# MecatronicaUSB/uw-slam

Hardware: AMD Instinct MI355X
Metric: frame-pair alignments/sec (640x480, 4 pyr lvls) (higher is better)
Workload: dtype f32; 1 GPU; synthetic 640x480 pairs, 4 pyramid levels (0..3), 10 GN iterations/level, no early exit, dense points, u16 depth plane, 1024 pairs in total, 1024 resident on rank 0 (128 distinct), image pyramids of both frames + depth pyramid and gradients of the reference frame + alignment per step; normal_equation_accumulation=f64, weights=identity, tuning=defaults, sampler=nearest, total_pairs=1024, pairs_on_rank0=1024

## Files before the change

### uw-slam_amd/csrc/uwt_kernels.h

```cpp
#pragma once

#include <hip/hip_runtime.h>
#include <stdint.h>

#include <type_traits>

#include "uwt_math.h"

namespace uwt {

constexpr int kBlock = 256;
constexpr int kAccFloats = 27;
constexpr int kRecWords = 64;
constexpr int kMaxSlices = 160;

constexpr int kArithOpenCV = 0, kArithLegacy = 1;

struct LevelK {
  int pitch;
  int iw, ih;
  int gw, gh;
  int n;
  int ng;
  float fx, fy, cx, cy, invfx, invfy;
// ... 903 lines not shown
};

__device__ __forceinline__ float sample_bilinear(const uint8_t* __restrict__ I2, const LevelK& L, float x, float y) {
  const float x0 = floorf(x), y0 = floorf(y);
  const float ax = x - x0, ay = y - y0;
  int ix0, iy0;
  asm("v_cvt_i32_f32 %0, %1" : "=v"(ix0) : "v"(x0));
  asm("v_cvt_i32_f32 %0, %1" : "=v"(iy0) : "v"(y0));
  asm("v_med3_i32 %0, %0, 0, %1" : "+v"(ix0) : "s"(L.iw - 1));
  asm("v_med3_i32 %0, %0, 0, %1" : "+v"(iy0) : "s"(L.ih - 1));
  const int ix1 = min(ix0 + 1, L.iw - 1), iy1 = min(iy0 + 1, L.ih - 1);
  const uint32_t r0 = __umul24((unsigned)iy0, (unsigned)L.pitch), r1 = __umul24((unsigned)iy1, (unsigned)L.pitch);
  const float a = (float)I2[r0 + (unsigned)ix0], b = (float)I2[r0 + (unsigned)ix1];
  const float c = (float)I2[r1 + (unsigned)ix0], d = (float)I2[r1 + (unsigned)ix1];
  const float top = __builtin_fmaf(ax, b - a, a);
  const float bot = __builtin_fmaf(ax, d - c, c);
  return __builtin_fmaf(ay, bot - top, top);
}

template <bool FINITE = false>
__device__ __forceinline__ float robust_weight(int mode, float rf, float inv_mad) {
  if (mode == kWeightsTukeyRef) {
    const float b = 4.6851f;
    const float inv_b2 = (float)(1.0 / (double)(b * b));
    const float x = rf * inv_mad;
    if (fabsf(x) <= b) {
      const float t = (float)(1.0 - (double)((x * x) * inv_b2));
      return t * t;
    }
    return 0.f;
  }
  if (mode == kWeightsHuber) {
    const float k = 1.345f;
    const float ax = fabsf(rf * inv_mad);
    if constexpr (FINITE) return ax <= k ? 1.0f : div_by<float>(k, ax, refined_rcp<float>(ax));
    return ax <= k ? 1.0f : k / ax;
  }
  return 1.0f;
}

struct WeightEntry {
  double rwd;
  double e;
  float w;
  float pad[3];
};
static_assert(sizeof(WeightEntry) == 32, "one ds_read_b32 (w) and, later, one ds_read_b128 (rwd, e) per pixel");
constexpr int kWeightTabBytes = 511 * (int)sizeof(WeightEntry);

__device__ __forceinline__ void fill_weight_table(WeightEntry* __restrict__ tab, int mode, float inv_mad, float gain) {
  for (int i = threadIdx.x; i < 511; i += kBlock) {
    const float rf = (float)(i - 255);
    const float w = robust_weight(mode, rf, inv_mad);
    const float rw1 = rf * w;
    WeightEntry t;
    t.w = w; t.pad[0] = t.pad[1] = t.pad[2] = 0.f;
    t.rwd = (double)((rf * gain) * w);
    t.e = (double)rf * (double)rw1;
    tab[i] = t;
  }
}

static __global__ __launch_bounds__(1024) void k_robust_weights(const float* __restrict__ r, int n, int kind, float* __restrict__ w,
                                                         float* __restrict__ out_stats) {
  __shared__ unsigned int hist[256];
  __shared__ float s_med, s_mad;
  auto median_of_hist = [&]() {
    const float m = (float)(n / 2);
    unsigned int bin = 0;
    float med = -1.0f;
    for (int i = 0; i < 256 && med < 0.0f; ++i) {
      bin += hist[i];
      if ((float)bin > m) med = (float)i;
    }
    return med;
  };
  for (int pass = 0; pass < 2; pass++) {
    for (int i = threadIdx.x; i < 256; i += blockDim.x) hist[i] = 0;
    __syncthreads();
    for (int i = threadIdx.x; i < n; i += blockDim.x) {
      const float v = pass == 0 ? r[i] : fabsf(r[i] - s_med);
      int q = (int)rintf(v);
      q = q < 0 ? 0 : (q > 255 ? 255 : q);
      atomicAdd(&hist[q], 1u);
    }
    __syncthreads();
    if (threadIdx.x == 0) {
      const float med = median_of_hist();
      if (pass == 0) s_med = med; else s_mad = 1.4826f * med;
    }
    __syncthreads();
  }
  if (threadIdx.x == 0) { out_stats[0] = s_med; out_stats[1] = s_mad; }
  if (!w) return;
  float mad = s_mad;
  if (mad == 0.0f) mad = 1.0f;
  const float inv_mad = (float)(1.0 / (double)mad);
  for (int i = threadIdx.x; i < n; i += blockDim.x) w[i] = robust_weight(kind, r[i], inv_mad);
}

struct TailUpdate {
  unsigned int* tickets;
  PairState* state;
  int* active;
  int on;
  int k, max_iters, early_exit, general, legacy_solve;
  float epsilon, gain;
};

struct ResidualArgs {
  const uint8_t* img;
  const int16_t* gx;
  const int16_t* gy;
  const uint16_t* depth;
  const int* ref_slots;
  const int* tgt_slots;
  const PairState* state;
  Pose pose;
  LevelK L;
  float zf, af;
  int groups_per_block;
  int slices;
  int pair_base;
  uint32_t* partials;
  const PairScale* scale;
  float gain;
  float* dumpJ;
  float* dumpR;
  uint8_t* dumpV;
  float* dumpW;
  int typed_loads;
  int stream_planes;
  int probe;
  TailUpdate tail;
};

struct CoreOverride {
  int groups_per_block;
  uint32_t* rec;
  const PairScale* scale = nullptr;
};

typedef float f4v __attribute__((ext_vector_type(4)));
typedef int i4v __attribute__((ext_vector_type(4)));
template <int VEC>
struct RefGroup {
  uint8_t i1[VEC];
  int16_t gx[VEC], gy[VEC];
  uint16_t dp[VEC];
  f4v gx4, gy4, dp4;
};

constexpr int kLoadsPlain = 0, kLoadsStream = 1, kLoadsTyped = 2;
template <int VEC, bool DEPTH, bool COMPUTE_ONLY = false, int STREAM = 0>
__device__ __forceinline__ void load_group(RefGroup<VEC>& r, const uint8_t* __restrict__ I1, const int16_t* __restrict__ GX,
                                           const int16_t* __restrict__ GY, const uint16_t* __restrict__ DP, uint32_t idx) {
  constexpr bool FAKE_PLANES = COMPUTE_ONLY;
  if constexpr (FAKE_PLANES) {
#pragma unroll
    for (int j = 0; j < VEC; j++) { r.i1[j] = (uint8_t)(idx + j); r.gx[j] = (int16_t)(idx * 3 + j); r.gy[j] = (int16_t)(idx * 5 - j); r.dp[j] = (uint16_t)(4000 + (idx & 255)); }
    return;
  }
  if constexpr (VEC == 4) {
    const uint32_t o2 = idx * 2u;
    if constexpr ((STREAM & kLoadsStream) != 0) {
      *reinterpret_cast<uint32_t*>(r.i1) = __builtin_nontemporal_load(reinterpret_cast<const uint32_t*>(I1 + idx));
      *reinterpret_cast<u2v*>(r.gx) = __builtin_nontemporal_load(reinterpret_cast<const u2v*>(reinterpret_cast<const uint8_t*>(GX) + o2));
      *reinterpret_cast<u2v*>(r.gy) = __builtin_nontemporal_load(reinterpret_cast<const u2v*>(reinterpret_cast<const uint8_t*>(GY) + o2));
      if constexpr (DEPTH) *reinterpret_cast<u2v*>(r.dp) = __builtin_nontemporal_load(reinterpret_cast<const u2v*>(reinterpret_cast<const uint8_t*>(DP) + o2));
    } else {
      *reinterpret_cast<uint32_t*>(r.i1) = *reinterpret_cast<const uint32_t*>(I1 + idx);
      *reinterpret_cast<uint2*>(r.gx) = *reinterpret_cast<const uint2*>(reinterpret_cast<const uint8_t*>(GX) + o2);
      *reinterpret_cast<uint2*>(r.gy) = *reinterpret_cast<const uint2*>(reinterpret_cast<const uint8_t*>(GY) + o2);
      if constexpr (DEPTH) *reinterpret_cast<uint2*>(r.dp) = *reinterpret_cast<const uint2*>(reinterpret_cast<const uint8_t*>(DP) + o2);
    }
  } else {
#pragma unroll
    for (int j = 0; j < VEC; j++) {
      r.i1[j] = I1[idx + j]; r.gx[j] = GX[idx + j]; r.gy[j] = GY[idx + j];
      if constexpr (DEPTH) r.dp[j] = DP[idx + j];
    }
  }
}

__device__ __forceinline__ i4v make_rsrc(const void* p, uint32_t bytes) {
  const unsigned long long b = (unsigned long long)p;
  i4v r;
  r.x = __builtin_amdgcn_readfirstlane((int)(unsigned)b);
  r.y = __builtin_amdgcn_readfirstlane((int)(unsigned)(b >> 32));
  r.z = __builtin_amdgcn_readfirstlane((int)bytes);
  r.w = __builtin_amdgcn_readfirstlane(0x00027FAC);
  return r;
}
struct TypedPlanes { const uint8_t* I1; i4v gx, gy, dp; };
template <bool DEPTH, bool NT>
__device__ __forceinline__ void load_group_typed(RefGroup<4>& r, const TypedPlanes& P, uint32_t idx) {
  const uint32_t o2 = idx * 2u;
  uint32_t& w = *reinterpret_cast<uint32_t*>(r.i1);
  if constexpr (NT) {
    asm volatile("global_load_dword %0, %1, %2 nt" : "+v"(w) : "v"(idx), "s"(P.I1));
    asm volatile("tbuffer_load_format_xyzw %0, %1, %2, 0 format:[BUF_DATA_FORMAT_16_16_16_16,BUF_NUM_FORMAT_SSCALED] offen nt" : "+v"(r.gx4) : "v"(o2), "s"(P.gx));
    asm volatile("tbuffer_load_format_xyzw %0, %1, %2, 0 format:[BUF_DATA_FORMAT_16_16_16_16,BUF_NUM_FORMAT_SSCALED] offen nt" : "+v"(r.gy4) : "v"(o2), "s"(P.gy));
    if constexpr (DEPTH) asm volatile("tbuffer_load_format_xyzw %0, %1, %2, 0 format:[BUF_DATA_FORMAT_16_16_16_16,BUF_NUM_FORMAT_SSCALED] offen nt" : "+v"(r.dp4) : "v"(o2), "s"(P.dp));
  } else {
    asm volatile("global_load_dword %0, %1, %2" : "+v"(w) : "v"(idx), "s"(P.I1));
    asm volatile("tbuffer_load_format_xyzw %0, %1, %2, 0 format:[BUF_DATA_FORMAT_16_16_16_16,BUF_NUM_FORMAT_SSCALED] offen" : "+v"(r.gx4) : "v"(o2), "s"(P.gx));
    asm volatile("tbuffer_load_format_xyzw %0, %1, %2, 0 format:[BUF_DATA_FORMAT_16_16_16_16,BUF_NUM_FORMAT_SSCALED] offen" : "+v"(r.gy4) : "v"(o2), "s"(P.gy));
    if constexpr (DEPTH) asm volatile("tbuffer_load_format_xyzw %0, %1, %2, 0 format:[BUF_DATA_FORMAT_16_16_16_16,BUF_NUM_FORMAT_SSCALED] offen" : "+v"(r.dp4) : "v"(o2), "s"(P.dp));
  }
}
template <bool DEPTH>
__device__ __forceinline__ void wait_planes_typed(RefGroup<4>& r) {
  uint32_t& w = *reinterpret_cast<uint32_t*>(r.i1);
  if constexpr (DEPTH) asm volatile("s_waitcnt vmcnt(0)" : "+v"(w), "+v"(r.gx4), "+v"(r.gy4), "+v"(r.dp4));
  else asm volatile("s_waitcnt vmcnt(0)" : "+v"(w), "+v"(r.gx4), "+v"(r.gy4));
}

template <int AR, int VEC, bool DEPTH, bool UNIT_FACTORS, bool DUMP, typename AccT, bool SQUARE = false, int SAMPLER = 0, int WEIGHTS = 0,
          bool COMPUTE_ONLY = false, int EXT_LDS = 0, int STREAM = 0, bool RAGGED = false>
__device__ __forceinline__ void residual_core(const ResidualArgs& a, const int pair, const int slice, const Pose& pose,
                                              unsigned char* lds, const RefGroup<VEC>* first = nullptr, int ref_slot = -1,
                                              int tgt_slot = -1, const CoreOverride* ov = nullptr);

template <int VEC, bool DEPTH, bool COMPUTE_ONLY>
__device__ __forceinline__ void load_first_group(RefGroup<VEC>& rg, const ResidualArgs& a, int ref_slot, int slice) {
  const size_t ref_off = (size_t)ref_slot * a.L.n;
  const int n_groups = a.L.ng / VEC;
  const int g = slice * a.groups_per_block + (int)threadIdx.x;
  load_group<VEC, DEPTH, COMPUTE_ONLY>(rg, a.img + ref_off, a.gx + ref_off, a.gy + ref_off, DEPTH ? a.depth + ref_off : nullptr,
                                       (uint32_t)min(g, n_groups - 1) * VEC);
}

template <int AR, int VEC, bool DEPTH, bool UNIT_FACTORS, bool DUMP, typename AccT, bool SQUARE = false, int SAMPLER = 0, int WEIGHTS = 0,
          bool COMPUTE_ONLY = false, int STREAM = 0, bool RAGGED = false>
__device__ __forceinline__ bool residual_block(const ResidualArgs& a, const int pair, const int slice) {
  Pose pose;
  if constexpr (COMPUTE_ONLY) {
    pose_identity(pose);
  } else if (a.state) {
    const PairState st = a.state[pair];
    if (st.level_done || st.status) return false;
    pose = st.pose;
  } else {
    pose = a.pose;
  }
  residual_core<AR, VEC, DEPTH, UNIT_FACTORS, DUMP, AccT, SQUARE, SAMPLER, WEIGHTS, COMPUTE_ONLY, 0, STREAM, RAGGED>(a, pair, slice, pose, nullptr);
  return true;
}

template <int AR, int VEC, bool DEPTH, bool UNIT_FACTORS, bool DUMP, typename AccT, bool SQUARE, int SAMPLER, int WEIGHTS, bool COMPUTE_ONLY,
          int EXT_LDS, int STREAM, bool RAGGED>
__device__ __forceinline__ void residual_core(const ResidualArgs& a, const int pair, const int slice, const Pose& pose,
                                              unsigned char* lds, const RefGroup<VEC>* first, int ref_slot, int tgt_slot,
                                              const CoreOverride* ov) {
  const int a_groups_per_block = ov ? ov->groups_per_block : a.groups_per_block;
  const bool a_probe = ov ? false : a.probe != 0;
  constexpr bool MASKED = std::is_same<AccT, double>::value && !DUMP;
  WarpK K;
  constexpr bool TD_LDS = AR == kArithOpenCV && !DUMP;
  __shared__ __attribute__((aligned(16))) double s_td[TD_LDS ? 12 : 2];
  if constexpr (TD_LDS) {
    warp_setup<kArithLegacy>(pose, K);
    if (threadIdx.x == 0) {
#pragma unroll
      for (int i = 0; i < 12; i++) s_td[i] = (double)K.T[i];
    }
    __syncthreads();
  } else {
    warp_setup<AR>(pose, K);
  }
  const LevelK L = a.L;
  if (ref_slot < 0) {
    ref_slot = a.ref_slots[pair];
    tgt_slot = a.tgt_slots[pair];
  }
  const size_t ref_off = (size_t)ref_slot * L.n, tgt_off = (size_t)tgt_slot * L.n;
  const uint8_t* __restrict__ I1 = a.img + ref_off;
  const uint8_t* __restrict__ I2 = a.img + tgt_off;
  const int16_t* __restrict__ GX = a.gx + ref_off;
  const int16_t* __restrict__ GY = a.gy + ref_off;
  const uint16_t* __restrict__ DP = DEPTH ? a.depth + ref_off : nullptr;

  __shared__ unsigned long long s_probe[2];
  if (a_probe && threadIdx.x == 0) {
    s_probe[0] = __builtin_amdgcn_s_memtime();
    s_probe[1] = __builtin_amdgcn_s_memrealtime();
  }
  AccT acc[kAccFloats];
#pragma unroll
  for (int i = 0; i < kAccFloats; i++) acc[i] = (AccT)0;
  uint32_t sum_r2 = 0, n_valid_wave = 0;
  double r2d = 0.0;
  constexpr bool GENERAL = SAMPLER != 0 || WEIGHTS != 0;
  AccT err = (AccT)0;
  float inv_mad = 1.f;
  if constexpr (WEIGHTS != 0) inv_mad = ov ? ov->scale->inv_mad : a.scale[pair].inv_mad;
  constexpr bool TABLE = WEIGHTS != 0 && SAMPLER == 0 && !DUMP;
  static_assert(!TABLE || EXT_LDS == 0, "the weighted path reduces in its own LDS");
  __shared__ __attribute__((aligned(16))) unsigned char tlds[TABLE ? kReduceLdsBytes : 16];
  static_assert(!TABLE || kWeightTabBytes <= kReduceLdsBytes, "table fits the reduction image");
  if constexpr (TABLE) {
    fill_weight_table(reinterpret_cast<WeightEntry*>(tlds), WEIGHTS, inv_mad, a.gain);
    __syncthreads();
  }

  const int n_groups = L.ng / VEC;
  const int g_begin = slice * a_groups_per_block;
  const int g_end = min(g_begin + a_groups_per_block, n_groups);
  const int iters = (g_end - g_begin + kBlock - 1) / kBlock;

  RefGroup<VEC> rg;
  int g = g_begin + (int)threadIdx.x;
  constexpr bool TYPED = (STREAM & kLoadsTyped) != 0;
  constexpr bool NT = (STREAM & kLoadsStream) != 0;
  static_assert(!TYPED || (VEC == 4 && std::is_same<AccT, double>::value && !DUMP && !COMPUTE_ONLY && SAMPLER == 0 && WEIGHTS == 0),
                "typed plane loads: the identity path's production shape");
  TypedPlanes TP;
  if constexpr (TYPED) {
    TP.I1 = I1;
    TP.gx = make_rsrc(GX, (uint32_t)L.n * 2u);
    TP.gy = make_rsrc(GY, (uint32_t)L.n * 2u);
    TP.dp = make_rsrc(DEPTH ? (const void*)DP : (const void*)GX, (uint32_t)L.n * 2u);
    *reinterpret_cast<uint32_t*>(rg.i1) = 0u;
    rg.gx4 = rg.gy4 = rg.dp4 = (f4v)(0.f);
    load_group_typed<DEPTH, NT>(rg, TP, (uint32_t)min(g, n_groups - 1) * VEC);
  } else if (first) rg = *first;
  else load_group<VEC, DEPTH, COMPUTE_ONLY, STREAM>(rg, I1, GX, GY, DP, (uint32_t)min(g, n_groups - 1) * VEC);
  const uint32_t idx0 = (uint32_t)g * VEC;
  const uint32_t y0 = __umulhi(idx0, L.magic);
  float yf = (float)y0, xf0 = (float)(idx0 - y0 * (uint32_t)L.pitch);
  const uint32_t step_y = __umulhi((uint32_t)(kBlock * VEC), L.magic);
  const float step_yf = (float)step_y, step_xf = (float)((uint32_t)(kBlock * VEC) - step_y * (uint32_t)L.pitch), wf = (float)L.pitch;
  constexpr int N = (VEC % 2 == 0) ? 2 : 1;
  using F = typename std::conditional<N == 2, v2f, float>::type;
  constexpr int NU = VEC / N;
  auto body = [&](RefGroup<VEC>& rg, const int ahead, RefGroup<VEC>& nxt) __attribute__((always_inline)) {
    const bool active = g < g_end;
    const unsigned long long active_mask = __builtin_amdgcn_sicmp(g, g_end, kIcmpSLT);
    constexpr bool TD_READ = TD_LDS;
    if constexpr (TD_READ) {
      unsigned off = 0;
      asm volatile("" : "+v"(off));
      const double* tdp = reinterpret_cast<const double*>(reinterpret_cast<const unsigned char*>(s_td) + off);
#pragma unroll
      for (int i = 0; i < 12; i++) K.Td[i] = tdp[i];
    }
    const uint32_t idx = (uint32_t)min(g, n_groups - 1) * VEC;
    if constexpr (TYPED) wait_planes_typed<DEPTH>(rg);
    uint8_t i1[VEC];
#pragma unroll
    for (int j = 0; j < VEC; j++) i1[j] = rg.i1[j];
    F x2[NU], y2[NU], iz[NU];
    unsigned long long okm[VEC];
    uint32_t gidx[VEC];
    unsigned long long colm[VEC];
#pragma unroll
    for (int j = 0; j < VEC; j++) colm[j] = active_mask;
    if constexpr (RAGGED) {
      const unsigned long long m_in = active_mask & __builtin_amdgcn_fcmpf(xf0, (float)L.gw, kFcmpOLT);
      const unsigned long long m_all = active_mask & __builtin_amdgcn_fcmpf(xf0, (float)(L.gw & ~3), kFcmpOLT);
      const int rem = L.gw & 3;
#pragma unroll
      for (int j = 0; j < VEC; j++) colm[j] = (VEC == 1 || j < rem) ? m_in : m_all;
    }
#pragma unroll
    for (int u = 0; u < NU; u++) {
      F z = bc<F>(1.0f), xf;
      unsigned long long okin[N];
      float dlow[N];
#pragma unroll
      for (int c = 0; c < N; c++) {
        const int j = u * N + c;
        okin[c] = colm[j];
        dlow[c] = 1.0f;
        if constexpr (DEPTH && TYPED) {
          const float d = rg.dp4[j];
          dlow[c] = d;
          put(z, c, d);
        } else if constexpr (DEPTH) {
          const int d = (int)(int16_t)rg.dp[j];
          dlow[c] = (float)d;
          if constexpr (!MASKED) okin[c] &= __builtin_amdgcn_sicmp(d, 0, kIcmpSGT);
          put(z, c, dlow[c]);
        }
        put(xf, c, (float)j);
      }
      if constexpr (DEPTH) z = z * bc<F>(L.zscale);
      xf = bc<F>(xf0) + xf;
      if constexpr (MASKED) {
        if constexpr (DEPTH) {
          F z2;
          warp_point<AR, F>(L, K, xf, bc<F>(yf), z, x2[u], y2[u], z2, iz[u]);
#pragma unroll
          for (int c = 0; c < N; c++) {
            const float uc = get(x2[u], c), vc = get(y2[u], c);
            float lo;
            asm("v_min3_f32 %0, %1, %2, %3" : "=v"(lo) : "v"(uc), "v"(vc), "v"(dlow[c]));
            okm[u * N + c] = okin[c] & __builtin_amdgcn_fcmpf(lo, 0.f, kFcmpOGT) & __builtin_amdgcn_fcmpf(vc, (float)L.ih, kFcmpOLT) &
                             __builtin_amdgcn_fcmpf(uc, (float)L.iw, kFcmpOLT);
          }
        } else {
          pixel_warp_raw<AR, F>(L, K, xf, bc<F>(yf), z, okin, x2[u], y2[u], iz[u], &okm[u * N]);
        }
#pragma unroll
        for (int c = 0; c < N; c++) {
          float r = get(iz[u], c);
          asm("v_max_f32 %0, 0, %0" : "+v"(r));
          put(iz[u], c, r);
          int ix2 = round_pos(get(x2[u], c)), iy2 = round_pos(get(y2[u], c));
          asm("v_med3_i32 %0, %0, 0, %1" : "+v"(ix2) : "s"(L.iw - 1));
          asm("v_med3_i32 %0, %0, 0, %1" : "+v"(iy2) : "s"(L.ih - 1));
          gidx[u * N + c] = __umul24((unsigned)iy2, (unsigned)L.pitch) + (unsigned)ix2;
        }
      } else {
        pixel_warp<AR, F>(L, K, xf, bc<F>(yf), z, okin, x2[u], y2[u], iz[u], &okm[u * N], &gidx[u * N]);
      }
    }
    int i2[VEC];
    float s2[VEC];
#pragma unroll
    for (int j = 0; j < VEC; j++) {
      constexpr bool FAKE_GATHER = COMPUTE_ONLY;
      if constexpr (FAKE_GATHER) i2[j] = (int)i1[j] + (int)(gidx[j] & 1);
      else if constexpr (TYPED) asm volatile("global_load_ubyte %0, %1, %2" : "=v"(i2[j]) : "v"(gidx[j]), "s"(I2));
      else if constexpr (SAMPLER == 0) i2[j] = I2[gidx[j]];
      else s2[j] = sample_bilinear(I2, L, get(x2[j / N], j % N), get(y2[j / N], j % N));
    }
    F g0[NU], g1[NU];
#pragma unroll
    for (int j = 0; j < VEC; j++) {
      if constexpr (MASKED) {
        float gxf, gyf;
        if constexpr (TYPED) { gxf = rg.gx4[j]; gyf = rg.gy4[j]; }
        else { gxf = (float)rg.gx[j]; gyf = (float)rg.gy[j]; }
        if constexpr (AR == kArithOpenCV && !TYPED) {
          asm("" : "+v"(gxf));
          asm("" : "+v"(gyf));
        }
        put(g0[j / N], j % N, gxf);
        put(g1[j / N], j % N, gyf);
      } else {
        put(g0[j / N], j % N, keep_f((float)rg.gx[j], okm[j]));
        put(g1[j / N], j % N, keep_f((float)rg.gy[j], okm[j]));
      }
    }
    __builtin_amdgcn_sched_barrier(0);
    if constexpr (TYPED) load_group_typed<DEPTH, NT>(nxt, TP, (uint32_t)min(g + ahead * kBlock, n_groups - 1) * VEC);
    else load_group<VEC, DEPTH, COMPUTE_ONLY, STREAM>(nxt, I1, GX, GY, DP, (uint32_t)min(g + ahead * kBlock, n_groups - 1) * VEC);
    __builtin_amdgcn_sched_barrier(0);
    auto gathers_landed = [&]() __attribute__((always_inline)) {
      if constexpr (TYPED) asm volatile("s_waitcnt vmcnt(%4)" : "+v"(i2[0]), "+v"(i2[1]), "+v"(i2[2]), "+v"(i2[3]) : "n"(DEPTH ? 4 : 3));
    };
    constexpr bool DIRECT = AR == kArithOpenCV && MASKED && !GENERAL;
    if constexpr (DIRECT) {
#pragma unroll
      for (int u = 0; u < NU; u++) {
        F a0, b1, av[4], bv[4];
        jw_terms<UNIT_FACTORS, SQUARE, F>(L, a.zf, a.af, x2[u], y2[u], iz[u], a0, b1, av, bv);
        const F j0 = g0[u] * a0, j1 = g1[u] * b1;
#pragma unroll
        for (int c = 0; c < N; c++) {
          const int j = u * N + c;
          double Jd[6];
          jacobian_row_f64<SQUARE, F>(g0[u], g1[u], j0, j1, av, bv, c, Jd);
          if (u == 0 && c == 0) gathers_landed();
          const int ri = i2[j] - (int)i1[j];
          masked_sums_lo(acc, Jd, okm[j]);
          masked_sums_hi<0>(acc, r2d, Jd, (double)ri, 0.0, okm[j]);
          n_valid_wave += (uint32_t)__builtin_popcountll(okm[j]);
          __builtin_amdgcn_sched_barrier(0);
        }
      }
    } else if constexpr (MASKED && GENERAL && !TABLE) {
#pragma unroll
      for (int u = 0; u < NU; u++) {
        if constexpr (SAMPLER != 0) {
          if (u == 0) {
#pragma unroll
            for (int j = 0; j < VEC; j++) asm volatile("" : "+v"(s2[j]));
          }
        }
        F a0, b1, av[4], bv[4], j0, j1, Ju[6];
        if constexpr (AR == kArithOpenCV) {
          jw_terms<UNIT_FACTORS, SQUARE, F>(L, a.zf, a.af, x2[u], y2[u], iz[u], a0, b1, av, bv);
          j0 = g0[u] * a0;
          j1 = g1[u] * b1;
        } else {
          pixel_jacobian<AR, UNIT_FACTORS, SQUARE, false, F>(L, a.zf, a.af, x2[u], y2[u], iz[u], g0[u], g1[u], Ju);
        }
#pragma unroll
        for (int c = 0; c < N; c++) {
          const int j = u * N + c;
          float Jp[6];
          if constexpr (AR == kArithOpenCV) jacobian_row_f32<SQUARE, F>(g0[u], g1[u], j0, j1, av, bv, c, Jp);
          else {
#pragma unroll
            for (int k = 0; k < 6; k++) Jp[k] = get(Ju[k], c);
          }
          float rf;
          if constexpr (SAMPLER == 0) rf = (float)(i2[j] - (int)i1[j]);
          else rf = s2[j] - (float)i1[j];
          const float w = robust_weight<true>(WEIGHTS, rf, inv_mad);
          double Jd[6];
#pragma unroll
          for (int k = 0; k < 6; k++) Jd[k] = (double)(w * Jp[k]);
          const double e = (double)rf * (double)(rf * w);
          masked_sums_lo(acc, Jd, okm[j]);
          masked_sums_hi<1>(acc, err, Jd, (double)((rf * a.gain) * w), e, okm[j]);
          n_valid_wave += (uint32_t)__builtin_popcountll(okm[j]);
          __builtin_amdgcn_sched_barrier(0);
        }
      }
    } else {
    F J[NU][6];
#pragma unroll
    for (int u = 0; u < NU; u++)
      pixel_jacobian<AR, UNIT_FACTORS, SQUARE, DUMP, F>(L, a.zf, a.af, x2[u], y2[u], iz[u], g0[u], g1[u], J[u]);
    __builtin_amdgcn_sched_barrier(0);
    gathers_landed();
    if constexpr (TABLE) {
#pragma unroll
      for (int u = 0; u < NU; u++) {
        uint32_t off[N];
        F wv;
#pragma unroll
        for (int c = 0; c < N; c++) {
          const int j = u * N + c;
          const int ri = i2[j] - (int)i1[j];
          n_valid_wave += (uint32_t)__builtin_popcountll(okm[j]);
          off[c] = (uint32_t)(ri + 255) * (uint32_t)sizeof(WeightEntry);
          put(wv, c, *reinterpret_cast<const float*>(tlds + off[c] + 16));
        }
#pragma unroll
        for (int k = 0; k < 6; k++) J[u][k] = wv * J[u][k];
#pragma unroll
        for (int c = 0; c < N; c++) {
          const int j = u * N + c;
          const double2 re = *reinterpret_cast<const double2*>(tlds + off[c]);
          if constexpr (MASKED) {
            double Jd[6];
#pragma unroll
            for (int k = 0; k < 6; k++) Jd[k] = (double)get(J[u][k], c);
            masked_sums_lo(acc, Jd, okm[j]);
            masked_sums_hi<1>(acc, err, Jd, re.x, re.y, okm[j]);
          } else {
            float Jp[6];
#pragma unroll
            for (int k = 0; k < 6; k++) Jp[k] = get(J[u][k], c);
            const unsigned long long m = okm[j];
            if (lane_bit(m)) {
              err += (AccT)re.y;
              accumulate_preweighted(acc, Jp, re.x);
            }
          }
        }
        __builtin_amdgcn_sched_barrier(0);
      }
    } else {
#pragma unroll
    for (int j = 0; j < VEC; j++) {
      float Jp[6];
#pragma unroll
      for (int k = 0; k < 6; k++) Jp[k] = get(J[j / N][k], j % N);
      int ri = 0;
      float rf_dump = 0.f, w_dump = 0.f;
      if constexpr (!GENERAL && MASKED) {
        ri = i2[j] - (int)i1[j];
        double Jd[6];
#pragma unroll
        for (int k = 0; k < 6; k++) Jd[k] = (double)Jp[k];
        masked_sums_lo(acc, Jd, okm[j]);
        masked_sums_hi<0>(acc, r2d, Jd, (double)ri, 0.0, okm[j]);
      } else if constexpr (!GENERAL) {
        ri = keep_i(i2[j] - (int)i1[j], okm[j]);
        accumulate(acc, Jp, ri);
      } else if constexpr (MASKED) {
        float rf;
        if constexpr (SAMPLER == 0) rf = (float)(i2[j] - (int)i1[j]);
        else rf = s2[j] - (float)i1[j];
        const float w = robust_weight<true>(WEIGHTS, rf, inv_mad);
        double Jd[6];
#pragma unroll
        for (int k = 0; k < 6; k++) Jd[k] = (double)(w * Jp[k]);
        const double e = (double)rf * (double)(rf * w);
        masked_sums_lo(acc, Jd, okm[j]);
        masked_sums_hi<1>(acc, err, Jd, (double)((rf * a.gain) * w), e, okm[j]);
      } else {
        float rf;
        if constexpr (SAMPLER == 0) rf = (float)keep_i(i2[j] - (int)i1[j], okm[j]);
        else rf = keep_f(s2[j] - (float)i1[j], okm[j]);
        const float w = robust_weight(WEIGHTS, rf, inv_mad);
        accumulate_weighted(acc, err, Jp, rf, w, a.gain);
        ri = (int)rintf(rf);
        if constexpr (DUMP) {
          rf_dump = rf;
          w_dump = w;
        }
      }
      if constexpr (GENERAL || !MASKED) sum_r2 += (uint32_t)__mul24(ri, ri);
      n_valid_wave += (uint32_t)__builtin_popcountll(okm[j]);
      if constexpr (DUMP) {
        if (active) {
          const size_t p = (size_t)pair * L.ng + idx + j;
          const bool ok = lane_bit(okm[j]);
          if (a.dumpV) a.dumpV[p] = ok ? 1 : 0;
          if constexpr (GENERAL) {
            if (a.dumpR) a.dumpR[p] = ok ? rf_dump : 0.f;
            if (a.dumpW) a.dumpW[p] = ok ? w_dump : 0.f;
            if (a.dumpJ)
              for (int k = 0; k < 6; k++) a.dumpJ[p * 6 + k] = ok ? Jp[k] : 0.f;
          } else {
            if (a.dumpR) a.dumpR[p] = (float)ri;
            if (a.dumpJ)
              for (int k = 0; k < 6; k++) a.dumpJ[p * 6 + k] = Jp[k];
          }
        }
      }
    }
    }
    }
    xf0 += step_xf;
    yf += step_yf;
    const bool wrap = xf0 >= wf;
    xf0 -= wrap ? wf : 0.f;
    yf += wrap ? 1.f : 0.f;
  };
  if constexpr (TYPED) {
    RefGroup<VEC> rgB;
    *reinterpret_cast<uint32_t*>(rgB.i1) = 0u;
    rgB.gx4 = rgB.gy4 = rgB.dp4 = (f4v)(0.f);
    for (int it = 0; it < iters; it += 2) {
      body(rg, 1, rgB);
      g += kBlock;
      if (it + 1 < iters) {
        body(rgB, 1, rg);
        g += kBlock;
      }
    }
    wait_planes_typed<DEPTH>(rg);
    wait_planes_typed<DEPTH>(rgB);
  } else {
    for (int it = 0; it < iters; it++, g += kBlock) body(rg, 1, rg);
  }
  const uint32_t n_valid = (threadIdx.x & 63) == 0 ? n_valid_wave : 0u;
  uint32_t* out_rec = ov ? ov->rec : a.partials + ((size_t)pair * a.slices + slice) * kRecWords;
  constexpr bool R2D = MASKED && !GENERAL;
  const bool coherent = !ov && a.tail.on != 0;
  if constexpr (EXT_LDS != 0 && R2D) block_reduce_store_at<AccT, false, EXT_LDS, double>(lds, acc, r2d, n_valid, out_rec, err);
  else if constexpr (EXT_LDS != 0) block_reduce_store_at<AccT, GENERAL, EXT_LDS>(lds, acc, sum_r2, n_valid, out_rec, err);
  else if constexpr (TABLE) {
    __syncthreads();
    block_reduce_store_at<AccT, true>(tlds, acc, sum_r2, n_valid, out_rec, err, coherent);
  } else if constexpr (R2D) block_reduce_store<AccT, false, double>(acc, r2d, n_valid, out_rec, err, coherent);
  else block_reduce_store<AccT, GENERAL>(acc, sum_r2, n_valid, out_rec, err, coherent);
  if (a_probe && threadIdx.x == 0) {
    uint32_t* rec = a.partials + ((size_t)pair * a.slices + slice) * kRecWords;
    rec[60] = (uint32_t)(__builtin_amdgcn_s_memtime() - s_probe[0]);
    rec[61] = (uint32_t)(__builtin_amdgcn_s_memrealtime() - s_probe[1]);
  }
}

__device__ __forceinline__ void tail_update_wave(const ResidualArgs& a, int pair);

template <int AR, int VEC, bool DEPTH, bool UNIT_FACTORS, bool DUMP, typename AccT, bool SQUARE = false, int SAMPLER = 0, int WEIGHTS = 0,
          bool COMPUTE_ONLY = false, int STREAM = 0, bool RAGGED = false>
__global__ __launch_bounds__(kBlock) void k_residual(const ResidualArgs a) {
  const int pair = (int)blockIdx.y + a.pair_base;
  const bool live = residual_block<AR, VEC, DEPTH, UNIT_FACTORS, DUMP, AccT, SQUARE, SAMPLER, WEIGHTS, COMPUTE_ONLY, STREAM, RAGGED>(a, pair, (int)blockIdx.x);
  if constexpr (!COMPUTE_ONLY && !DUMP) {
    if (a.tail.on && live && threadIdx.x < 64) tail_update_wave(a, pair);
  }
}

template <int AR, int VEC, bool DEPTH, bool UNIT_FACTORS, bool DUMP, typename AccT, bool SQUARE = false, int SAMPLER = 0, int WEIGHTS = 0,
          int STREAM = 0, bool RAGGED = false>
__global__ __launch_bounds__(kBlock) __attribute__((amdgpu_waves_per_eu(4, 4))) void k_residual_w4(const ResidualArgs a) {
  const int pair = (int)blockIdx.y + a.pair_base;
  const bool live = residual_block<AR, VEC, DEPTH, UNIT_FACTORS, DUMP, AccT, SQUARE, SAMPLER, WEIGHTS, false, STREAM, RAGGED>(a, pair, (int)blockIdx.x);
  if constexpr (!DUMP) {
    if (a.tail.on && live && threadIdx.x < 64) tail_update_wave(a, pair);
  }
}

struct GeneralArgs {
  int sampler;
  int weights;
  float gain;
  unsigned int* hist;
  PairScale* scale;
};

__device__ __forceinline__ int first_crossing(const unsigned int v[8], float m, int lane) {
  unsigned int tot = 0;
#pragma unroll
  for (int k = 0; k < 8; k++) tot += v[k];
  unsigned int inc = tot;
#pragma unroll
  for (int d = 1; d < 64; d <<= 1) {
    const unsigned int up = __shfl_up(inc, d, 64);
    if (lane >= d) inc += up;
  }
  unsigned int cum = inc - tot;
  int idx = 0x7fffffff;
#pragma unroll
  for (int k = 0; k < 8; k++) {
    cum += v[k];
    if (idx == 0x7fffffff && (float)cum > m) idx = lane * 8 + k;
  }
#pragma unroll
  for (int d = 32; d > 0; d >>= 1) idx = min(idx, __shfl_xor(idx, d, 64));
  return idx;
}

__device__ __forceinline__ PairScale wave_scale(const unsigned int mine[8], unsigned int* __restrict__ h, bool tukey, int lane) {
  unsigned int n = 0;
#pragma unroll
  for (int k = 0; k < 8; k++) {
    h[lane * 8 + k] = mine[k];
    n += mine[k];
  }
  __builtin_amdgcn_wave_barrier();
#pragma unroll
  for (int d = 32; d > 0; d >>= 1) n += __shfl_xor(n, d, 64);
  const float m = (float)(n / 2);
  int med;
  {
    unsigned int v[8];
    if (tukey) {
      unsigned int neg = 0;
#pragma unroll
      for (int k = 0; k < 8; k++) neg += (lane * 8 + k <= 255) ? mine[k] : 0u;
#pragma unroll
      for (int d = 32; d > 0; d >>= 1) neg += __shfl_xor(neg, d, 64);
#pragma unroll
      for (int k = 0; k < 8; k++) {
        const int t = lane * 8 + k;
        v[k] = t == 0 ? neg : (t <= 255 ? h[t + 255] : 0u);
      }
      const int idx = first_crossing(v, m, lane);
      med = idx == 0x7fffffff ? 255 : idx;
    } else {
      const int idx = first_crossing(mine, m, lane);
      med = idx == 0x7fffffff ? 255 : idx - 255;
    }
  }
  const int dmax = tukey ? 255 : 510;
  int dmed;
  {
    unsigned int v[8];
#pragma unroll
    for (int k = 0; k < 8; k++) {
      const int d = lane * 8 + k;
      unsigned int c = 0;
      if (d < dmax) {
        const int lo = med - d, hi = med + d;
        if (lo >= -255 && lo <= 255) c += h[lo + 255];
        if (d > 0 && hi <= 255 && hi >= -255) c += h[hi + 255];
      }
      v[k] = c;
    }
    const int idx = first_crossing(v, m, lane);
    dmed = idx == 0x7fffffff ? dmax : idx;
  }
  PairScale sc;
  sc.med0 = (float)med;
  sc.n_valid = (int)n;
  sc.pad = 0;
  float mad = 1.4826f * (float)dmed;
  if (!n || mad == 0.f) mad = 1.f;
  sc.inv_mad = (float)(1.0 / (double)mad);
  return sc;
}

static __global__ __launch_bounds__(256) void k_scale_stage(const GeneralArgs ga, const PairState* state, int n_pairs, int pair_base) {
  __shared__ unsigned int sh[4][kHistBins];
  const int wave = threadIdx.x >> 6, lane = threadIdx.x & 63;
  const int i = blockIdx.x * 4 + wave;
  if (i >= n_pairs) return;
  const int pair = i + pair_base;
  const PairState st = state[pair];
  if (st.level_done || st.status) return;
  const unsigned int* gh = ga.hist + (size_t)pair * kHistBins;
  unsigned int mine[8];
#pragma unroll
  for (int k = 0; k < 8; k++) {
    const int b = lane * 8 + k;
    mine[k] = b < 511 ? gh[b] : 0u;
  }
  const PairScale sc = wave_scale(mine, sh[wave], ga.weights == kWeightsTukeyRef, lane);
  if (lane == 0) ga.scale[pair] = sc;
}

constexpr int kHistRep = 8;
constexpr int kHistTicketWord = kHistBins - 1;

// ... 1276 lines not shown
```

Baseline: 69090 alignments/s.

## Rotate residual loop into front/back stages to overlap gathers with next group's warp

```diff
diff --git a/uw-slam_amd/csrc/uwt_kernels.h b/uw-slam_amd/csrc/uwt_kernels.h
--- a/uw-slam_amd/csrc/uwt_kernels.h
+++ b/uw-slam_amd/csrc/uwt_kernels.h
@@ -1079,6 +1079,10 @@
 };
 
 constexpr int kLoadsPlain = 0, kLoadsStream = 1, kLoadsTyped = 2;
+#ifndef UWT_RESIDUAL_ROTATE
+#define UWT_RESIDUAL_ROTATE 1
+#endif
+constexpr bool kResidualRotate = UWT_RESIDUAL_ROTATE != 0;
 template <int VEC, bool DEPTH, bool COMPUTE_ONLY = false, int STREAM = 0>
 __device__ __forceinline__ void load_group(RefGroup<VEC>& r, const uint8_t* __restrict__ I1, const int16_t* __restrict__ GX,
                                            const int16_t* __restrict__ GY, const uint16_t* __restrict__ DP, uint32_t idx) {
@@ -1120,27 +1124,45 @@
   return r;
 }
 struct TypedPlanes { const uint8_t* I1; i4v gx, gy, dp; };
-template <bool DEPTH, bool NT>
-__device__ __forceinline__ void load_group_typed(RefGroup<4>& r, const TypedPlanes& P, uint32_t idx) {
-  const uint32_t o2 = idx * 2u;
+template <bool NT>
+__device__ __forceinline__ void load_grads_typed(RefGroup<4>& r, const TypedPlanes& P, uint32_t idx, uint32_t o2) {
   uint32_t& w = *reinterpret_cast<uint32_t*>(r.i1);
   if constexpr (NT) {
     asm volatile("global_load_dword %0, %1, %2 nt" : "+v"(w) : "v"(idx), "s"(P.I1));
     asm volatile("tbuffer_load_format_xyzw %0, %1, %2, 0 format:[BUF_DATA_FORMAT_16_16_16_16,BUF_NUM_FORMAT_SSCALED] offen nt" : "+v"(r.gx4) : "v"(o2), "s"(P.gx));
     asm volatile("tbuffer_load_format_xyzw %0, %1, %2, 0 format:[BUF_DATA_FORMAT_16_16_16_16,BUF_NUM_FORMAT_SSCALED] offen nt" : "+v"(r.gy4) : "v"(o2), "s"(P.gy));
-    if constexpr (DEPTH) asm volatile("tbuffer_load_format_xyzw %0, %1, %2, 0 format:[BUF_DATA_FORMAT_16_16_16_16,BUF_NUM_FORMAT_SSCALED] offen nt" : "+v"(r.dp4) : "v"(o2), "s"(P.dp));
   } else {
     asm volatile("global_load_dword %0, %1, %2" : "+v"(w) : "v"(idx), "s"(P.I1));
     asm volatile("tbuffer_load_format_xyzw %0, %1, %2, 0 format:[BUF_DATA_FORMAT_16_16_16_16,BUF_NUM_FORMAT_SSCALED] offen" : "+v"(r.gx4) : "v"(o2), "s"(P.gx));
     asm volatile("tbuffer_load_format_xyzw %0, %1, %2, 0 format:[BUF_DATA_FORMAT_16_16_16_16,BUF_NUM_FORMAT_SSCALED] offen" : "+v"(r.gy4) : "v"(o2), "s"(P.gy));
-    if constexpr (DEPTH) asm volatile("tbuffer_load_format_xyzw %0, %1, %2, 0 format:[BUF_DATA_FORMAT_16_16_16_16,BUF_NUM_FORMAT_SSCALED] offen" : "+v"(r.dp4) : "v"(o2), "s"(P.dp));
-  }
+  }
+}
+template <bool NT>
+__device__ __forceinline__ void load_depth_typed(RefGroup<4>& r, const TypedPlanes& P, uint32_t o2) {
+  if constexpr (NT) asm volatile("tbuffer_load_format_xyzw %0, %1, %2, 0 format:[BUF_DATA_FORMAT_16_16_16_16,BUF_NUM_FORMAT_SSCALED] offen nt" : "+v"(r.dp4) : "v"(o2), "s"(P.dp));
+  else asm volatile("tbuffer_load_format_xyzw %0, %1, %2, 0 format:[BUF_DATA_FORMAT_16_16_16_16,BUF_NUM_FORMAT_SSCALED] offen" : "+v"(r.dp4) : "v"(o2), "s"(P.dp));
+}
+template <bool DEPTH, bool NT>
+__device__ __forceinline__ void load_group_typed(RefGroup<4>& r, const TypedPlanes& P, uint32_t idx) {
+  const uint32_t o2 = idx * 2u;
+  load_grads_typed<NT>(r, P, idx, o2);
+  if constexpr (DEPTH) load_depth_typed<NT>(r, P, o2);
 }
 template <bool DEPTH>
 __device__ __forceinline__ void wait_planes_typed(RefGroup<4>& r) {
   uint32_t& w = *reinterpret_cast<uint32_t*>(r.i1);
   if constexpr (DEPTH) asm volatile("s_waitcnt vmcnt(0)" : "+v"(w), "+v"(r.gx4), "+v"(r.gy4), "+v"(r.dp4));
   else asm volatile("s_waitcnt vmcnt(0)" : "+v"(w), "+v"(r.gx4), "+v"(r.gy4));
+}
+
+template <int YOUNGER>
+__device__ __forceinline__ void wait_depth_typed(RefGroup<4>& r) {
+  asm volatile("s_waitcnt vmcnt(%1)" : "+v"(r.dp4) : "n"(YOUNGER));
+}
+template <int YOUNGER>
+__device__ __forceinline__ void wait_back_typed(RefGroup<4>& r, int (&i2)[4]) {
+  uint32_t& w = *reinterpret_cast<uint32_t*>(r.i1);
+  asm volatile("s_waitcnt vmcnt(%7)" : "+v"(w), "+v"(r.gx4), "+v"(r.gy4), "+v"(i2[0]), "+v"(i2[1]), "+v"(i2[2]), "+v"(i2[3]) : "n"(YOUNGER));
 }
 
 template <int AR, int VEC, bool DEPTH, bool UNIT_FACTORS, bool DUMP, typename AccT, bool SQUARE = false, int SAMPLER = 0, int WEIGHTS = 0,
@@ -1242,6 +1264,9 @@
   constexpr bool NT = (STREAM & kLoadsStream) != 0;
   static_assert(!TYPED || (VEC == 4 && std::is_same<AccT, double>::value && !DUMP && !COMPUTE_ONLY && SAMPLER == 0 && WEIGHTS == 0),
                 "typed plane loads: the identity path's production shape");
+  constexpr bool DIRECT = AR == kArithOpenCV && MASKED && !GENERAL;
+  constexpr bool ROTATED = DIRECT && (TYPED || COMPUTE_ONLY) && kResidualRotate;
+  constexpr int kFrontLoads = (DEPTH ? 1 : 0) + VEC + 3;
   TypedPlanes TP;
   if constexpr (TYPED) {
     TP.I1 = I1;
@@ -1250,7 +1275,7 @@
     TP.dp = make_rsrc(DEPTH ? (const void*)DP : (const void*)GX, (uint32_t)L.n * 2u);
     *reinterpret_cast<uint32_t*>(rg.i1) = 0u;
     rg.gx4 = rg.gy4 = rg.dp4 = (f4v)(0.f);
-    load_group_typed<DEPTH, NT>(rg, TP, (uint32_t)min(g, n_groups - 1) * VEC);
+    if constexpr (!ROTATED) load_group_typed<DEPTH, NT>(rg, TP, (uint32_t)min(g, n_groups - 1) * VEC);
   } else if (first) rg = *first;
   else load_group<VEC, DEPTH, COMPUTE_ONLY, STREAM>(rg, I1, GX, GY, DP, (uint32_t)min(g, n_groups - 1) * VEC);
   const uint32_t idx0 = (uint32_t)g * VEC;
@@ -1261,8 +1286,48 @@
   constexpr int N = (VEC % 2 == 0) ? 2 : 1;
   using F = typename std::conditional<N == 2, v2f, float>::type;
   constexpr int NU = VEC / N;
-  auto body = [&](RefGroup<VEC>& rg, const int ahead, RefGroup<VEC>& nxt) __attribute__((always_inline)) {
+  struct Carry {
+    F x2[NU], y2[NU], iz[NU], g0[NU], g1[NU];
+    uint8_t i1[VEC];
+    int i2[VEC];
+    float s2[VEC];
+    unsigned long long okm[VEC];
+    uint32_t idx;
+    bool active;
+  };
+  auto take_planes = [&](RefGroup<VEC>& rg, Carry& cy) __attribute__((always_inline)) {
+#pragma unroll
+    for (int j = 0; j < VEC; j++) {
+      cy.i1[j] = rg.i1[j];
+      if constexpr (MASKED) {
+        float gxf, gyf;
+        if constexpr (TYPED) { gxf = rg.gx4[j]; gyf = rg.gy4[j]; }
+        else { gxf = (float)rg.gx[j]; gyf = (float)rg.gy[j]; }
+        if constexpr (AR == kArithOpenCV && !TYPED) {
+          asm("" : "+v"(gxf));
+          asm("" : "+v"(gyf));
+        }
+        put(cy.g0[j / N], j % N, gxf);
+        put(cy.g1[j / N], j % N, gyf);
+      } else {
+        put(cy.g0[j / N], j % N, keep_f((float)rg.gx[j], cy.okm[j]));
+        put(cy.g1[j / N], j % N, keep_f((float)rg.gy[j], cy.okm[j]));
+      }
+    }
+  };
+  constexpr int kLone = -1;
+  uint32_t o2_ahead = 0;
+  auto group_o2 = [&](int gg) __attribute__((always_inline)) { return (uint32_t)min(gg, n_groups - 1) * (uint32_t)(VEC * 2); };
+  auto request_depth = [&](RefGroup<VEC>& r, uint32_t o2) __attribute__((always_inline)) {
+    if constexpr (TYPED) {
+      if constexpr (DEPTH) load_depth_typed<NT>(r, TP, o2);
+    } else {
+      load_group<VEC, DEPTH, COMPUTE_ONLY, STREAM>(r, I1, GX, GY, DP, o2 >> 1);
+    }
+  };
+  auto front = [&](RefGroup<VEC>& rg, const int ahead, RefGroup<VEC>& nxt, Carry& cy, auto head) __attribute__((always_inline)) {
     const bool active = g < g_end;
+    cy.active = active;
     const unsigned long long active_mask = __builtin_amdgcn_sicmp(g, g_end, kIcmpSLT);
     constexpr bool TD_READ = TD_LDS;
     if constexpr (TD_READ) {
@@ -1272,13 +1337,23 @@
 #pragma unroll
       for (int i = 0; i < 12; i++) K.Td[i] = tdp[i];
     }
-    const uint32_t idx = (uint32_t)min(g, n_groups - 1) * VEC;
-    if constexpr (TYPED) wait_planes_typed<DEPTH>(rg);
-    uint8_t i1[VEC];
-#pragma unroll
-    for (int j = 0; j < VEC; j++) i1[j] = rg.i1[j];
-    F x2[NU], y2[NU], iz[NU];
-    unsigned long long okm[VEC];
+    if constexpr (!ROTATED) cy.idx = (uint32_t)min(g, n_groups - 1) * VEC;
+    else cy.idx = 0;
+    constexpr bool LONE = decltype(head)::value == kLone;
+    uint32_t o2 = o2_ahead;
+    if constexpr (LONE) {
+      o2 = group_o2(g);
+      request_depth(rg, o2);
+    }
+    if constexpr (TYPED && ROTATED) {
+      if constexpr (DEPTH) wait_depth_typed<LONE ? 0 : decltype(head)::value>(rg);
+    } else if constexpr (TYPED) wait_planes_typed<DEPTH>(rg);
+    if constexpr (ROTATED && !LONE) {
+      o2_ahead = group_o2(g + ahead * kBlock);
+      request_depth(nxt, o2_ahead);
+    }
+    F (&x2)[NU] = cy.x2, (&y2)[NU] = cy.y2, (&iz)[NU] = cy.iz;
+    unsigned long long (&okm)[VEC] = cy.okm;
     uint32_t gidx[VEC];
     unsigned long long colm[VEC];
 #pragma unroll
@@ -1343,42 +1418,44 @@
         pixel_warp<AR, F>(L, K, xf, bc<F>(yf), z, okin, x2[u], y2[u], iz[u], &okm[u * N], &gidx[u * N]);
       }
     }
-    int i2[VEC];
-    float s2[VEC];
+    const uint32_t idx_next = ROTATED ? 0u : (uint32_t)min(g + ahead * kBlock, n_groups - 1) * VEC;
+    int (&i2)[VEC] = cy.i2;
+    float (&s2)[VEC] = cy.s2;
 #pragma unroll
     for (int j = 0; j < VEC; j++) {
       constexpr bool FAKE_GATHER = COMPUTE_ONLY;
-      if constexpr (FAKE_GATHER) i2[j] = (int)i1[j] + (int)(gidx[j] & 1);
+      if constexpr (FAKE_GATHER) i2[j] = (int)rg.i1[j] + (int)(gidx[j] & 1);
       else if constexpr (TYPED) asm volatile("global_load_ubyte %0, %1, %2" : "=v"(i2[j]) : "v"(gidx[j]), "s"(I2));
       else if constexpr (SAMPLER == 0) i2[j] = I2[gidx[j]];
       else s2[j] = sample_bilinear(I2, L, get(x2[j / N], j % N), get(y2[j / N], j % N));
     }
-    F g0[NU], g1[NU];
-#pragma unroll
-    for (int j = 0; j < VEC; j++) {
-      if constexpr (MASKED) {
-        float gxf, gyf;
-        if constexpr (TYPED) { gxf = rg.gx4[j]; gyf = rg.gy4[j]; }
-        else { gxf = (float)rg.gx[j]; gyf = (float)rg.gy[j]; }
-        if constexpr (AR == kArithOpenCV && !TYPED) {
-          asm("" : "+v"(gxf));
-          asm("" : "+v"(gyf));
-        }
-        put(g0[j / N], j % N, gxf);
-        put(g1[j / N], j % N, gyf);
-      } else {
-        put(g0[j / N], j % N, keep_f((float)rg.gx[j], okm[j]));
-        put(g1[j / N], j % N, keep_f((float)rg.gy[j], okm[j]));
-      }
-    }
+    if constexpr (ROTATED) {
+      if constexpr (TYPED) load_grads_typed<NT>(rg, TP, o2 >> 1, o2);
+      __builtin_amdgcn_sched_barrier(0);
+      return;
+    }
+    take_planes(rg, cy);
     __builtin_amdgcn_sched_barrier(0);
-    if constexpr (TYPED) load_group_typed<DEPTH, NT>(nxt, TP, (uint32_t)min(g + ahead * kBlock, n_groups - 1) * VEC);
-    else load_group<VEC, DEPTH, COMPUTE_ONLY, STREAM>(nxt, I1, GX, GY, DP, (uint32_t)min(g + ahead * kBlock, n_groups - 1) * VEC);
+    if constexpr (TYPED) load_group_typed<DEPTH, NT>(nxt, TP, idx_next);
+    else load_group<VEC, DEPTH, COMPUTE_ONLY, STREAM>(nxt, I1, GX, GY, DP, idx_next);
     __builtin_amdgcn_sched_barrier(0);
-    auto gathers_landed = [&]() __attribute__((always_inline)) {
-      if constexpr (TYPED) asm volatile("s_waitcnt vmcnt(%4)" : "+v"(i2[0]), "+v"(i2[1]), "+v"(i2[2]), "+v"(i2[3]) : "n"(DEPTH ? 4 : 3));
-    };
-    constexpr bool DIRECT = AR == kArithOpenCV && MASKED && !GENERAL;
+  };
+  auto gathers_landed = [&](Carry& cy) __attribute__((always_inline)) {
+    if constexpr (TYPED) asm volatile("s_waitcnt vmcnt(%4)" : "+v"(cy.i2[0]), "+v"(cy.i2[1]), "+v"(cy.i2[2]), "+v"(cy.i2[3]) : "n"(DEPTH ? 4 : 3));
+  };
+  auto wait_back = [&](RefGroup<VEC>& rg, Carry& cy, auto younger) __attribute__((always_inline)) {
+    if constexpr (TYPED) wait_back_typed<decltype(younger)::value>(rg, cy.i2);
+  };
+  auto back = [&](RefGroup<VEC>& rg, Carry& cy) __attribute__((always_inline)) {
+    if constexpr (ROTATED) take_planes(rg, cy);
+    F (&x2)[NU] = cy.x2, (&y2)[NU] = cy.y2, (&iz)[NU] = cy.iz, (&g0)[NU] = cy.g0, (&g1)[NU] = cy.g1;
+    uint8_t (&i1)[VEC] = cy.i1;
+    int (&i2)[VEC] = cy.i2;
+    float (&s2)[VEC] = cy.s2;
+    unsigned long long (&okm)[VEC] = cy.okm;
+    const bool active = cy.active;
+    const uint32_t idx = cy.idx;
+    (void)s2; (void)active; (void)idx;
     if constexpr (DIRECT) {
 #pragma unroll
       for (int u = 0; u < NU; u++) {
@@ -1390,7 +1467,7 @@
           const int j = u * N + c;
           double Jd[6];
           jacobian_row_f64<SQUARE, F>(g0[u], g1[u], j0, j1, av, bv, c, Jd);
-          if (u == 0 && c == 0) gathers_landed();
+          if (!ROTATED && u == 0 && c == 0) gathers_landed(cy);
           const int ri = i2[j] - (int)i1[j];
           masked_sums_lo(acc, Jd, okm[j]);
           masked_sums_hi<0>(acc, r2d, Jd, (double)ri, 0.0, okm[j]);
@@ -1444,7 +1521,7 @@
     for (int u = 0; u < NU; u++)
       pixel_jacobian<AR, UNIT_FACTORS, SQUARE, DUMP, F>(L, a.zf, a.af, x2[u], y2[u], iz[u], g0[u], g1[u], J[u]);
     __builtin_amdgcn_sched_barrier(0);
-    gathers_landed();
+    gathers_landed(cy);
     if constexpr (TABLE) {
 #pragma unroll
       for (int u = 0; u < NU; u++) {
@@ -1546,28 +1623,80 @@
     }
     }
     }
+  };
+  auto advance = [&]() __attribute__((always_inline)) {
     xf0 += step_xf;
     yf += step_yf;
     const bool wrap = xf0 >= wf;
     xf0 -= wrap ? wf : 0.f;
     yf += wrap ? 1.f : 0.f;
+    g += kBlock;
+    if constexpr (ROTATED) asm("" : "+v"(g));
   };
-  if constexpr (TYPED) {
+  using std::integral_constant;
+  auto body = [&](RefGroup<VEC>& rg, const int ahead, RefGroup<VEC>& nxt) __attribute__((always_inline)) {
+    Carry cy;
+    front(rg, ahead, nxt, cy, integral_constant<int, 0>());
+    back(rg, cy);
+    advance();
+  };
+  if constexpr (ROTATED) {
+    RefGroup<VEC> rgB;
+    if constexpr (TYPED) {
+      *reinterpret_cast<uint32_t*>(rgB.i1) = 0u;
+      rgB.gx4 = rgB.gy4 = rgB.dp4 = (f4v)(0.f);
+    }
+    Carry cA, cB;
+#pragma unroll
+    for (int j = 0; j < VEC; j++) cA.i2[j] = cB.i2[j] = 0;
+    const integral_constant<int, 0> all;
+    const integral_constant<int, kLone> lone;
+    const integral_constant<int, kFrontLoads - 1> head;
+    const integral_constant<int, kFrontLoads> younger;
+    if (iters & 1) {
+      front(rg, 1, rgB, cA, lone);
+      advance();
+      wait_back(rg, cA, all);
+      back(rg, cA);
+    }
+    if (iters >= 2) {
+      o2_ahead = group_o2(g);
+      request_depth(rg, o2_ahead);
+      front(rg, 1, rgB, cA, all);
+      advance();
+      for (int it = iters & 1; it + 2 < iters; it += 2) {
+        front(rgB, 1, rg, cB, head);
+        advance();
+        wait_back(rg, cA, younger);
+        back(rg, cA);
+        front(rg, 1, rgB, cA, head);
+        advance();
+        wait_back(rgB, cB, younger);
+        back(rgB, cB);
+      }
+      front(rgB, 1, rg, cB, head);
+      advance();
+      wait_back(rg, cA, younger);
+      back(rg, cA);
+      wait_back(rgB, cB, all);
+      back(rgB, cB);
+    }
+    if constexpr (TYPED) {
+      wait_planes_typed<DEPTH>(rg);
+      wait_planes_typed<DEPTH>(rgB);
+    }
+  } else if constexpr (TYPED) {
     RefGroup<VEC> rgB;
     *reinterpret_cast<uint32_t*>(rgB.i1) = 0u;
     rgB.gx4 = rgB.gy4 = rgB.dp4 = (f4v)(0.f);
     for (int it = 0; it < iters; it += 2) {
       body(rg, 1, rgB);
-      g += kBlock;
-      if (it + 1 < iters) {
-        body(rgB, 1, rg);
-        g += kBlock;
-      }
+      if (it + 1 < iters) body(rgB, 1, rg);
     }
     wait_planes_typed<DEPTH>(rg);
     wait_planes_typed<DEPTH>(rgB);
   } else {
-    for (int it = 0; it < iters; it++, g += kBlock) body(rg, 1, rg);
+    for (int it = 0; it < iters; it++) body(rg, 1, rg);
   }
   const uint32_t n_valid = (threadIdx.x & 63) == 0 ? n_valid_wave : 0u;
   uint32_t* out_rec = ov ? ov->rec : a.partials + ((size_t)pair * a.slices + slice) * kRecWords;
```

Result: slower. 68280 alignments/s (-1.2%).
